# dernasherbrezon/sdr-server

Hardware: AMD Instinct MI355X
Metric: input IQ Msamples/s processed (all clients), 2.016 Msps->48 kHz xlating FIR (higher is better)
Workload: dtype f32; 1 GPU; 1024 clients x 48 kHz off one 2.016 Msps cu8 stream, D=42, 505 taps, 262144-byte blocks (BASELINE configs[3]; N=1: the >=1000-client single-GPU target); clients_total=1024, clients_per_gpu=1024, blocks_per_call=8, mode=optimized, parallelism=single GPU, rccl_ranks=1, feed=xlating_multi (C host)

## Files before the change

sdr-server_amd/csrc/xl_kernels.hip:

```cpp
#include "xl_dev_inline.h"
#include "xl_chain_plan.h"

#include <hip/hip_ext.h>

#include <stdlib.h>

__global__ __launch_bounds__(64) void xl_nco_table_kernel(const XlNcoClient *__restrict__ cl, uint32_t n,
                                                          const float2 *state_in, float2 *state_out,
                                                          float2 *__restrict__ tab, const XlPos pos,
                                                          const uint32_t explicit_K, const uint32_t prio,
                                                          const uint32_t lanes) {
  if (prio == 3) __builtin_amdgcn_s_setprio(3);
  else if (prio == 2) __builtin_amdgcn_s_setprio(2);
  else if (prio == 1) __builtin_amdgcn_s_setprio(1);
  if (threadIdx.x >= lanes) return;
  const uint32_t c = blockIdx.x * lanes + threadIdx.x;
  if (c >= n) return;
  const XlNcoClient k = cl[c];
  const XlBnd bnd = xl_nco_bnd(k, pos, explicit_K);
  asm volatile("" ::: "v255", "a255");
  xl_nco_client_chain<true>(k, bnd, 0u, bnd.K, state_in, state_out, tab);
}

#define XLC_RING 64u
XL_DEV uint32_t xl_lds_off(const void *p) { return (uint32_t)(uintptr_t)(__attribute__((address_space(3))) const char *)p; }
XL_DEV void xl_lds_post(const uint32_t addr, const uint32_t v) { asm volatile("ds_write_b32 %0, %1" ::"v"(addr), "v"(v) : "memory"); }
XL_DEV void xl_lds_post64(const uint32_t addr, const v2f v) { asm volatile("ds_write_b64 %0, %1" ::"v"(addr), "v"(v) : "memory"); }
XL_DEV uint32_t xl_lds_poll(const uint32_t addr) {
  uint32_t v;
  asm volatile("ds_read_b32 %0, %1\n\ts_waitcnt lgkmcnt(0)" : "=v"(v) : "v"(addr) : "memory");
  return v;
}

XL_DEV uint32_t xl_lds_poll3_min(const uint32_t a0, const uint32_t a1, const uint32_t a2) {
  uint32_t v0, v1, v2;
  asm volatile("ds_read_b32 %0, %3\n\tds_read_b32 %1, %4\n\tds_read_b32 %2, %5\n\ts_waitcnt lgkmcnt(0)"
               : "=&v"(v0), "=&v"(v1), "=&v"(v2)
               : "v"(a0), "v"(a1), "v"(a2)
               : "memory");
  v0 = v0 < v1 ? v0 : v1;
  return v0 < v2 ? v0 : v2;
}
XL_DEV uint32_t xl_chain_lim(const uint32_t mn) { return mn >= 0x7FFFFFE0u ? 0xFFFFFFFFu : 2u * mn + XLC_RING; }
XL_DEV uint32_t xl_chain_wait_drained(const uint32_t upto, const uint32_t a0, const uint32_t a1, const uint32_t a2) {
  uint32_t lim = 0u;
  for (uint32_t spin = 0; spin < (1u << 22); ++spin) {
    lim = xl_chain_lim((uint32_t)__builtin_amdgcn_readfirstlane((int)xl_lds_poll3_min(a0, a1, a2)));
    if (upto <= lim) break;
    __builtin_amdgcn_s_sleep(1);
  }
  return lim;
}
XL_DEV uint32_t xl_chain_event(uint32_t ev) {
  const unsigned long long act = __ballot(ev != 0xFFFFFFFFu);
  if (act == 0ull) return 0xFFFFFFFFu;
  const uint32_t first = (uint32_t)__builtin_amdgcn_readlane((int)ev, (int)__ffsll((long long)act) - 1);
  if (__ballot(ev != 0xFFFFFFFFu && ev != first) == 0ull) return first;
#pragma unroll
  for (int sh = 1; sh < 64; sh <<= 1) {
    const uint32_t other = (uint32_t)__shfl_xor((int)ev, sh);
    ev = other < ev ? other : ev;
  }
  return (uint32_t)__builtin_amdgcn_readfirstlane((int)ev);
}

#define XLC_ALIGN ".p2align 6\n\t"
#define XLC_MUL "v_pk_mul_f32 %[t1], %[p], %[inc] op_sel_hi:[1,0]\n\tv_pk_mul_f32 %[t2], %[p], %[inc] op_sel:[0,1] op_sel_hi:[1,1]\n\t"
#define XLC_ADD "v_pk_add_f32 %[p], %[t1], %[t2] op_sel:[0,1] op_sel_hi:[1,0] neg_lo:[0,1]\n\t"
#define XLC_STEP XLC_MUL XLC_ADD
#define XLC_STEP2(I1, I2) XLC_MUL I1 "\n\t" XLC_ADD I2 "\n\t"
#define XLC_STEPS10 XLC_STEP XLC_STEP XLC_STEP XLC_STEP XLC_STEP XLC_STEP XLC_STEP XLC_STEP XLC_STEP XLC_STEP
#define XLC_ANY_LOOP                                                                       \
  "1:\n\t" XLC_MUL "ds_write_b64 %[addr], %[p]\n\t" XLC_ADD                               \
  XLC_STEP2("v_add_u32 %[cnt], 1, %[cnt]", "s_sub_u32 %[todo], %[todo], 1")               \
  XLC_MUL "ds_write_b32 %[paddr], %[cnt]\n\t" XLC_ADD                                     \
  XLC_MUL "v_add_u32 %[off], 0x200, %[off]\n\t" XLC_ADD                                   \
  XLC_MUL "v_and_b32 %[off], 0x7fff, %[off]\n\t" XLC_ADD                                  \
  XLC_STEP2("v_add_u32 %[addr], %[off], %[base]", "s_cmp_lg_u32 %[todo], 0")              \
  XLC_STEPS10 "s_cbranch_scc1 1b\n\t"
#define XLC_B8_LOOP                                                                        \
  "2:\n\t" XLC_E7("0", "512", "1024", "1536", "2048", "2560", "3072")                    \
  XLC_MUL "ds_write_b64 %[addr], %[p] offset:3584\n\t" XLC_ADD                           \
  XLC_STEP2("v_add_u32 %[cnt], 8, %[cnt]", "s_sub_u32 %[todo8], %[todo8], 1")            \
  XLC_MUL "ds_write_b32 %[paddr], %[cnt]\n\t" XLC_ADD                                    \
  XLC_MUL "v_add_u32 %[off], 0x1000, %[off]\n\t" XLC_ADD                                 \
  XLC_MUL "v_and_b32 %[off], 0x7fff, %[off]\n\t" XLC_ADD                                 \
  XLC_STEP2("v_add_u32 %[addr], %[off], %[base]", "s_cmp_lg_u32 %[todo8], 0")            \
  XLC_STEPS10 "s_cbranch_scc1 2b\n\t"
#define XLC_ANY_PART "s_cmp_eq_u32 %[todo], 0\n\ts_cbranch_scc1 3f\n\t" XLC_ANY_LOOP "3:\n\ts_nop 0\n\t"
#define XLC_B8_PART "s_cmp_eq_u32 %[todo8], 0\n\ts_cbranch_scc1 4f\n\t" XLC_B8_LOOP "4:\n\ts_nop 0\n\t"
#define XLC_STEP_LOOP "1:\n\t" XLC_STEP2("s_sub_u32 %[todo], %[todo], 1", "s_cmp_lg_u32 %[todo], 0") "s_cbranch_scc1 1b\n\t"
#define XLC_QENTRY(OFFS) XLC_MUL "ds_write_b64 %[addr], %[p] offset:" OFFS "\n\t" XLC_ADD XLC_STEP XLC_STEP
#define XLC_E(OFFS) XLC_QENTRY(OFFS) XLC_STEP XLC_STEP XLC_STEP XLC_STEPS10
#define XLC_E7(B0, B1, B2, B3, B4, B5, B6) XLC_E(B0) XLC_E(B1) XLC_E(B2) XLC_E(B3) XLC_E(B4) XLC_E(B5) XLC_E(B6)
#define XLC_E8(B0, B1, B2, B3, B4, B5, B6, B7) XLC_E7(B0, B1, B2, B3, B4, B5, B6) XLC_E(B7)
#define XLC_B32_LOOP                                                                                         \
  XLC_E8("0", "512", "1024", "1536", "2048", "2560", "3072", "3584")                                       \
  XLC_E8("4096", "4608", "5120", "5632", "6144", "6656", "7168", "7680")                                   \
  XLC_E8("8192", "8704", "9216", "9728", "10240", "10752", "11264", "11776")                               \
  XLC_E("12288") XLC_E("12800") XLC_E("13312") XLC_E("13824") XLC_E("14336") XLC_E("14848")               \
  XLC_QENTRY("15360")                                                                                      \
  XLC_MUL "ds_read_b32 %[mn], %[an0]\n\t" XLC_ADD                                                           \
  XLC_MUL "ds_read_b32 %[n1], %[an1]\n\t" XLC_ADD                                                           \
  XLC_MUL "ds_read_b32 %[n2], %[an2]\n\t" XLC_ADD XLC_STEPS10                                               \
  XLC_MUL "ds_write_b64 %[addr], %[p] offset:15872\n\t" XLC_ADD                                             \
  XLC_MUL "v_add_u32 %[cnt], 32, %[cnt]\n\t" XLC_ADD "s_sub_u32 %[todo], %[todo], 1\n\t"                    \
  XLC_MUL "ds_write_b32 %[paddr], %[cnt]\n\t" XLC_ADD                                                       \
  XLC_MUL "v_add_u32 %[off], 0x4000, %[off]\n\t" XLC_ADD                                                    \
  XLC_MUL "v_and_b32 %[off], 0x7fff, %[off]\n\t" XLC_ADD                                                    \
  XLC_STEP2("v_add_u32 %[addr], %[off], %[base]", "s_add_u32 %[need], %[need], 16")                         \
  XLC_STEP2("s_waitcnt lgkmcnt(0)", "v_min_u32 %[mn], %[mn], %[n1]")                                        \
  XLC_STEP2("v_min_u32 %[mn], %[mn], %[n2]", "s_nop 0")                                                     \
  XLC_STEP2("v_readfirstlane_b32 %[sm], %[mn]", "s_nop 0")                                                  \
  XLC_STEP2("s_cmp_ge_u32 %[sm], %[need]", "s_cselect_b32 %[st], %[todo], 0")                               \
  XLC_STEP XLC_STEP XLC_STEP XLC_STEP XLC_STEP XLC_STEP
static_assert(XL_PH_STRIDE == 16u && XLC_RING * 64u * 8u == 0x8000u, "the chain wave's asm blocks are written for 16 steps per entry and a 32 KB ring");

__global__ __launch_bounds__(256) void xl_nco_chain_kernel(const XlNcoClient *__restrict__ cl, uint32_t n,
                                                           const float2 *state_in, const XlChainCalls calls,
                                                           XlPos pos, unsigned long long *stats) {
  asm volatile("" ::: "v255", "a255");
  const unsigned long long t_entry = stats ? wall_clock64() : 0ull;
  __shared__ v2f ring[XLC_RING][64];
  __shared__ uint32_t s_emax;
  __shared__ uint32_t s_prod;
  __shared__ uint32_t s_next[3];
  const uint32_t w = __builtin_amdgcn_readfirstlane(threadIdx.x >> 6), lane = threadIdx.x & 63u;
  const uint32_t c = blockIdx.x * 64u + lane;
  const bool have = c < n;
  XlNcoClient k;
  k.incr = make_float2(1.0f, 0.0f);
  k.out_off = 0u, k.slot = 0u, k.D = 1u, k.rem0 = 0u;
  if (have) k = cl[c];
  v2f p = {1.0f, 0.0f};
  if (w == 0 && have) p = (v2f){state_in[k.slot].x, state_in[k.slot].y};
  unsigned long long cyc = 0ull, ticks = 0ull, wfirst = 0ull;
  uint32_t entries = 0u;
  for (uint32_t call = 0; call < calls.n; ++call, pos = xl_grid_next(pos)) {
    float2 *const tab = calls.tab[call];
    float2 *const state_out = calls.state_out[call];
    if (call) __syncthreads();
    XlBnd bnd = xl_nco_bnd(k, pos, 0xFFFFFFFFu);
    if (!have) bnd.K = 0u;
    const uint32_t K = bnd.K, E = (K + XL_PH_STRIDE - 1u) >> XL_PH_SHIFT;
    if (threadIdx.x == 0) {
      s_emax = 0u;
      s_prod = 0u;
      s_next[0] = 0u, s_next[1] = 1u, s_next[2] = 2u;
    }
    __syncthreads();
    if (w == 0 && E > 0u) atomicMax(&s_emax, E);
    __syncthreads();
    const uint32_t Emax = (uint32_t)__builtin_amdgcn_readfirstlane((int)s_emax);
    const uint32_t a_prod = xl_lds_off(&s_prod), a_ring0 = xl_lds_off(&ring[0][0]), a_ring = xl_lds_off(&ring[0][lane]);
    v2f *__restrict__ o = reinterpret_cast<v2f *>(tab) + (k.out_off >> XL_PH_SHIFT);
    if (w == 0) {
      __builtin_amdgcn_s_setprio(3);
      const v2f inc = {k.incr.x, k.incr.y};
      uint32_t nb = xl_bnd_next(bnd, 0u);
      const uint32_t a_n0 = xl_lds_off(&s_next[0]), a_n1 = xl_lds_off(&s_next[1]), a_n2 = xl_lds_off(&s_next[2]);
      const unsigned long long c0 = stats ? clock64() : 0ull, w0 = stats ? wall_clock64() : 0ull;
      unsigned long long t_region = 0ull, t_drain = 0ull, t_b32 = 0ull;
      uint32_t n_drain = 0u, n_b32 = 0u, n_event = 0u, n_runs = 0u;
      uint32_t e = 0;
      uint32_t lim = XLC_RING;
      uint32_t evs = xl_chain_event(0u < K ? (nb < K ? nb : K) : 0xFFFFFFFFu);
      while (e < Emax) {
        uint32_t e_stop = evs == 0u ? 0u : (evs - 1u) >> XL_PH_SHIFT;
        e_stop = e_stop < Emax ? e_stop : Emax;
        if (pos.pad & XL_POS_FMA_STEP) e_stop = e;
        const unsigned long long r0 = stats ? clock64() : 0ull;
        if ((e << XL_PH_SHIFT) < K) {
          const XlChainPlan8 pl = xl_chain_plan8(e, e_stop, XLC_RING, 32u, 8u);
          uint32_t ee = e;
          v2f t1, t2;
#define XLC_COVER_RUN(N1, N8, PARTS)                                                                                         \
  if ((N1) + (N8) != 0u) {                                                                                                   \
    uint32_t todo = (N1), todo8 = (N8);                                                                                      \
    const uint32_t total = todo + 8u * todo8;                                                                                \
    if (ee + total > lim) {                                                                                                  \
      const unsigned long long d0 = stats ? clock64() : 0ull;                                                                \
      lim = xl_chain_wait_drained(ee + total, a_n0, a_n1, a_n2);                                                             \
      if (stats) t_drain += clock64() - d0, ++n_drain;                                                                       \
    }                                                                                                                        \
    uint32_t off = ((ee & (XLC_RING - 1u)) << 9) + lane * (uint32_t)sizeof(v2f);     \
    uint32_t addr = a_ring0 + off, cnt = ee;                                                                                 \
    ee += total;                                                                                                             \
    asm volatile(XLC_ALIGN PARTS                                                                                             \
                 : [p] "+v"(p), [off] "+v"(off), [addr] "+v"(addr), [cnt] "+v"(cnt), [t1] "=&v"(t1), [t2] "=&v"(t2),         \
                   [todo] "+s"(todo), [todo8] "+s"(todo8)                                                                    \
                 : [inc] "v"(inc), [base] "v"(a_ring0), [paddr] "v"(a_prod)                                                  \
                 : "memory", "scc");                                                                                         \
  }
          XLC_COVER_RUN(pl.head1, pl.head8, XLC_ANY_PART XLC_B8_PART);
          for (uint32_t want = pl.blocks; want != 0u;) {
            if (ee + 32u > lim) {
              const unsigned long long d0 = stats ? clock64() : 0ull;
              lim = xl_chain_wait_drained(ee + 32u, a_n0, a_n1, a_n2);
              if (stats) t_drain += clock64() - d0, ++n_drain;
            }
            uint32_t off = ((ee & (XLC_RING - 1u)) << 9) + lane * (uint32_t)sizeof(v2f);
            uint32_t addr = a_ring0 + off, cnt = ee;
            uint32_t left = want, need = (ee >> 1) - 16u, mn, n1, n2, sm, st;
            const unsigned long long b0 = stats ? clock64() : 0ull;
            asm volatile(XLC_ALIGN "1:\n\t" XLC_B32_LOOP "s_cmp_lg_u32 %[st], 0\n\ts_cbranch_scc1 1b\n\t"
                         : [p] "+v"(p), [off] "+v"(off), [addr] "+v"(addr), [cnt] "+v"(cnt), [t1] "=&v"(t1), [t2] "=&v"(t2),
                           [mn] "=&v"(mn), [n1] "=&v"(n1), [n2] "=&v"(n2), [todo] "+s"(left), [need] "+s"(need), [sm] "=&s"(sm),
                           [st] "=&s"(st)
                         : [inc] "v"(inc), [base] "v"(a_ring0), [paddr] "v"(a_prod), [an0] "v"(a_n0), [an1] "v"(a_n1), [an2] "v"(a_n2)
                         : "memory", "scc");
            const uint32_t ran = (want - left) << 5;
            if (stats) t_b32 += clock64() - b0, n_b32 += ran, ++n_runs;
            lim = xl_chain_lim(sm);
            ee += ran;
            want = left;
          }
          XLC_COVER_RUN(pl.tail1, pl.tail8, XLC_B8_PART XLC_ANY_PART);
#undef XLC_COVER_RUN
        }
        if (e_stop > e) e = e_stop;
        if (stats) t_region += clock64() - r0, ++n_event;
        if (e < Emax) {
          if (e + 1u > lim) lim = xl_chain_wait_drained(e + 1u, a_n0, a_n1, a_n2);
          const uint32_t m0 = e << XL_PH_SHIFT;
          if (m0 < K) xl_lds_post64(a_ring + (e & (XLC_RING - 1u)) * 64u * (uint32_t)sizeof(v2f), p);
          xl_lds_post(a_prod, e + 1u);
          uint32_t m = m0;
          if (!(pos.pad & XL_POS_FMA_STEP) && evs - m0 - 1u < XL_PH_STRIDE &&
              __ballot(m0 < K && (nb != evs || m0 + XL_PH_STRIDE > K)) == 0ull && m0 < K) {
            v2f t1, t2;
            uint32_t todo = evs - m0;
            asm volatile(XLC_ALIGN XLC_STEP_LOOP
                         : [p] "+v"(p), [t1] "=&v"(t1), [t2] "=&v"(t2), [todo] "+s"(todo)
                         : [inc] "v"(inc)
                         : "scc");
            p = xl_nco_renorm(p);
            nb = xl_bnd_next(bnd, evs);
            m = evs;
            todo = m0 + XL_PH_STRIDE - evs;
            if (todo != 0u && __ballot(nb <= m0 + XL_PH_STRIDE) == 0ull) {
              asm volatile(XLC_ALIGN XLC_STEP_LOOP
                           : [p] "+v"(p), [t1] "=&v"(t1), [t2] "=&v"(t2), [todo] "+s"(todo)
                           : [inc] "v"(inc)
                           : "scc");
              m = m0 + XL_PH_STRIDE;
            }
          }
          for (; m < m0 + XL_PH_STRIDE && m < K; ++m) {
            p = xl_nco_next_any(p, inc, bnd.flags);
            if (m + 1u == nb) {
              p = xl_nco_renorm(p);
              nb = xl_bnd_next(bnd, m + 1u);
            }
          }
          ++e;
          evs = xl_chain_event((e << XL_PH_SHIFT) < K ? (nb < K ? nb : K) : 0xFFFFFFFFu);
        }
      }
      if (have) state_out[k.slot] = make_float2(p.x, p.y);
      if (stats) {
        cyc += clock64() - c0;
        const unsigned long long w1 = wall_clock64();
        ticks += w1 - w0;
        entries += Emax;
        if (call == 0u) wfirst = w0;
        if (lane == 0u && blockIdx.x < 1024u) {
          stats[8192u + 8u * blockIdx.x + 1u + 2u * call] = w0 - t_entry;
          stats[8192u + 8u * blockIdx.x + 2u + 2u * call] = w1 - t_entry;
        }
        if (lane == 0u && blockIdx.x < 128u) {
          unsigned long long *const sp = stats + 4096u + 32u * blockIdx.x + 8u * call;
          const unsigned long long k0 = clock64(), k1 = clock64(), k2 = clock64(), k3 = clock64(), k4 = clock64();
          (void)k1, (void)k2, (void)k3;
          sp[0] = k0 - c0, sp[1] = t_region, sp[2] = t_drain, sp[3] = t_b32;
          sp[4] = n_drain, sp[5] = n_b32, sp[6] = n_event | ((unsigned long long)n_runs << 32), sp[7] = (k4 - k0) / 4ull;
        }
      }
      continue;
    }
    const uint32_t j = w - 1u;
    const uint32_t a_next = xl_lds_off(&s_next[j]);
    v4f *__restrict__ o4 = reinterpret_cast<v4f *>(o);
    for (uint32_t q = j; 2u * q < Emax; q += 3u) {
      const uint32_t need = 2u * q + 2u < Emax ? 2u * q + 2u : Emax;
      for (uint32_t spin = 0; spin < (1u << 24); ++spin) {
        if (xl_lds_poll(a_prod) >= need) break;
        __builtin_amdgcn_s_sleep(1);
      }
      if (2u * q < E) {
        v2f a, b2 = {0.0f, 0.0f};
        const uint32_t ra = a_ring + ((2u * q) & (XLC_RING - 1u)) * 64u * (uint32_t)sizeof(v2f);
        const uint32_t rb = a_ring + ((2u * q + 1u) & (XLC_RING - 1u)) * 64u * (uint32_t)sizeof(v2f);
        const bool two = 2u * q + 1u < E;
        asm volatile("ds_read_b64 %0, %1" : "=v"(a) : "v"(ra) : "memory");
        if (two) asm volatile("ds_read_b64 %0, %1" : "=v"(b2) : "v"(rb) : "memory");
        asm volatile("s_waitcnt lgkmcnt(0)" ::: "memory");
        if (two) o4[q] = (v4f){a.x, a.y, b2.x, b2.y};
        else o[2u * q] = a;
      }
      xl_lds_post(a_next, q + 3u);
    }
    xl_lds_post(a_next, 0xFFFFFFFFu);
  }
  if (stats) __syncthreads();
  if (stats && threadIdx.x == 0u) {
    if (blockIdx.x < 1024u) {
      stats[8192u + 8u * blockIdx.x] = t_entry;
      stats[8192u + 8u * blockIdx.x + 7u] = wall_clock64() - t_entry;
    }
    stats[4u * blockIdx.x] = cyc;
    stats[4u * blockIdx.x + 1u] = ticks;
    stats[4u * blockIdx.x + 2u] = entries;
    stats[4u * blockIdx.x + 3u] = wfirst;
  }
}

template <int FMT>
XL_DEV void xl_stage_window(const XlFirArgs &a, const uint32_t zero_below, const uint32_t win0, const uint32_t wlen,
                            v2f *__restrict__ win) {
  const uint32_t bd = blockDim.x;
  for (uint32_t j0 = threadIdx.x; j0 < wlen; j0 += 4u * bd) {
    v2f v[4];
    bool ok[4];
#pragma unroll
    for (int u = 0; u < 4; ++u) {
      const uint32_t j = j0 + u * bd;
      const uint32_t s = win0 + j;
      const bool first = s < a.n0;
      ok[u] = j < wlen && s >= zero_below && (first || s - a.n0 < a.n1);
      const void *src = (first || !ok[u]) ? a.in0 : a.in1;
      const uint32_t idx = ok[u] ? (first ? s : s - a.n0) : 0u;
      v[u] = xl_sample(src, FMT, idx);
    }
#pragma unroll
    for (int u = 0; u < 4; ++u) {
      const uint32_t j = j0 + u * bd;
      if (j < wlen) win[j] = ok[u] ? v[u] : (v2f){0.0f, 0.0f};
    }
  }
}

template <int CT, int MODE, bool WIDE>
__global__ __launch_bounds__(64 * XL_NW_MAX) __attribute__((amdgpu_num_sgpr(96))) void xl_fir_kernel(const XlFirArgs a) {
  extern __shared__ __attribute__((aligned(16))) v2f xl_win[];
  const uint32_t OT = a.ota;

  if (blockIdx.x < a.nco_blocks) {
    if (((a.flags >> 4) & 3u) == 3u) __builtin_amdgcn_s_setprio(3);
    else if (((a.flags >> 4) & 3u) == 2u) __builtin_amdgcn_s_setprio(2);
    else if (((a.flags >> 4) & 3u) == 1u) __builtin_amdgcn_s_setprio(1);
    const uint32_t nwave = threadIdx.x >> 6, nlane = threadIdx.x & 63u;
    if (nwave < a.nco_wpw && nlane < XL_NCO_LANES) {
      const unsigned long long t0 = a.trace ? wall_clock64() : 0ull;
      const uint32_t c = (blockIdx.x * a.nco_wpw + nwave) * XL_NCO_LANES + nlane;
      if (c < a.nco_nclients) {
        const XlNcoClient k = a.nco_clients[c];
        const XlBnd bnd = xl_nco_bnd(k, xl_grid_next(a.pos), 0xFFFFFFFFu);
        xl_nco_client_chain<false>(k, bnd, 0u, bnd.K, a.nco_state_in, a.nco_state_out, a.nco_tab);
      }
      if (a.trace && nlane == 0) {
        unsigned long long *tn = a.trace + ((size_t)blockIdx.x * XL_NW_MAX + nwave) * 6;
        tn[0] = t0;
        tn[3] = wall_clock64();
        tn[4] = __builtin_amdgcn_s_getreg((4 << 0) | (0 << 6) | (31 << 11));
        tn[5] = __builtin_amdgcn_s_getreg((20 << 0) | (0 << 6) | (31 << 11));
      }
    }
    return;
  }

  if (!(a.flags & 2u)) __builtin_amdgcn_s_setprio(3);
  const uint32_t b = blockIdx.x - a.nco_blocks;
  const unsigned long long t_entry = a.trace ? wall_clock64() : 0ull;

  const uint32_t roll_blocks = gridDim.x - a.nco_blocks < XL_ROLL_BLOCKS ? gridDim.x - a.nco_blocks : XL_ROLL_BLOCKS;
  if (a.hist_out != nullptr && b < roll_blocks) {
    const uint16_t *__restrict__ h0 = reinterpret_cast<const uint16_t *>(a.in0);
    const uint16_t *__restrict__ h1 = reinterpret_cast<const uint16_t *>(a.in1);
    uint16_t *__restrict__ ho = reinterpret_cast<uint16_t *>(a.hist_out);
    const uint32_t hu = a.hist_units, nu = a.block_units;
    for (uint32_t j = b * blockDim.x + threadIdx.x; j < hu; j += roll_blocks * blockDim.x) {
      const uint32_t sidx = nu + j;
      ho[j] = (sidx < hu) ? h0[sidx] : h1[sidx - hu];
    }
  }
  const uint32_t xcd = b & 7u, idx = b >> 3;
  const uint32_t total = a.ngroups * a.xtiles;
  const uint32_t per = total >> 3, extra = total & 7u;
// ... 131 lines not shown
    if (m < K && lane < OT) {
#pragma unroll
      for (int c = 0; c < CT; ++c) {
        if ((uint32_t)c < ncl) out[t[2 + c] + m] = xl_rotate<MODE>(acc[c].value(), phs[c]);
      }
    }
  }
  if (tr && lane == 0) {
    __builtin_amdgcn_s_waitcnt(0);
    tr[3] = wall_clock64();
  }
}

size_t xl_fir_lds_bytes_ota(uint32_t D, uint32_t Tpad, uint32_t ota) {
  return ((size_t)(ota - 1u) * D + Tpad) * sizeof(v2f);
}

uint32_t xl_fir_pick_ota(uint32_t D, uint32_t Tpad, size_t budget) {
  for (uint32_t ota = 64; ota >= 8; ota >>= 1)
    if (xl_fir_lds_bytes_ota(D, Tpad, ota) <= budget) return ota;
  return 0;
}

template <int CT, int MODE, bool WIDE>
static hipError_t xl_fir_go2(int nw, const XlFirArgs &a, size_t lds, hipStream_t s) {
  static bool attr_done = false;
  if (!attr_done) {
    hipError_t e = hipFuncSetAttribute(reinterpret_cast<const void *>(&xl_fir_kernel<CT, MODE, WIDE>),
                                       hipFuncAttributeMaxDynamicSharedMemorySize, 160 * 1024);
    if (e != hipSuccess) return e;
    attr_done = true;
  }
  const uint32_t nblocks = a.nco_blocks + 8u * ((a.ngroups * a.xtiles + 7u) / 8u);
  if (nblocks == 0) return hipSuccess;
  const size_t need = (size_t)nw * CT * 64u * sizeof(float2);
  if (lds < need) lds = need;
  hipLaunchKernelGGL((xl_fir_kernel<CT, MODE, WIDE>), dim3(nblocks), dim3(64 * nw), lds, s, a);
  return hipGetLastError();
}

template <int CT, int MODE>
static hipError_t xl_fir_go(int nw, const XlFirArgs &a, size_t lds, hipStream_t s) {
  return (a.flags & 1u) ? xl_fir_go2<CT, MODE, true>(nw, a, lds, s) : xl_fir_go2<CT, MODE, false>(nw, a, lds, s);
}

hipError_t xl_launch_fir(int ct, int mode, int nw, const XlFirArgs &a, size_t lds, hipStream_t s) {
  if (lds > 160 * 1024 || nw < 1 || nw > XL_NW_MAX) return hipErrorInvalidValue;
  if (a.ota != 64 && a.ota != 32 && a.ota != 16 && a.ota != 8) return hipErrorInvalidValue;
  switch (ct * 2 + (mode ? 1 : 0)) {
    case 2: return xl_fir_go<1, 0>(nw, a, lds, s);
    case 3: return xl_fir_go<1, 1>(nw, a, lds, s);
    case 4: return xl_fir_go<2, 0>(nw, a, lds, s);
    case 5: return xl_fir_go<2, 1>(nw, a, lds, s);
    case 8: return xl_fir_go<4, 0>(nw, a, lds, s);
    case 9: return xl_fir_go<4, 1>(nw, a, lds, s);
    case 16: return xl_fir_go<8, 0>(nw, a, lds, s);
    case 17: return xl_fir_go<8, 1>(nw, a, lds, s);
    case 18: return xl_fir_go<9, 0>(nw, a, lds, s);
    case 19: return xl_fir_go<9, 1>(nw, a, lds, s);
    case 20: return xl_fir_go<10, 0>(nw, a, lds, s);
    case 21: return xl_fir_go<10, 1>(nw, a, lds, s);
    case 24: return xl_fir_go<12, 0>(nw, a, lds, s);
    case 25: return xl_fir_go<12, 1>(nw, a, lds, s);
    default: return hipErrorInvalidValue;
  }
}

hipError_t xl_launch_nco_table(const XlNcoClient *clients, uint32_t nclients, const float2 *state_in,
                               float2 *state_out, float2 *phtab, XlPos pos, uint32_t explicit_K, uint32_t prio,
                               hipStream_t s) {
  if (nclients == 0) return hipSuccess;
  const uint32_t lanes = XL_NCO_LANES;
  hipLaunchKernelGGL(xl_nco_table_kernel, dim3((nclients + lanes - 1) / lanes), dim3(64), 0, s, clients, nclients,
                     state_in, state_out, phtab, pos, explicit_K, prio, lanes);
  return hipGetLastError();
}

hipError_t xl_launch_nco_chain(const XlNcoClient *clients, uint32_t nclients, const float2 *state_in,
                               const XlChainCalls &calls, XlPos pos, unsigned long long *stats, hipStream_t s,
                               hipEvent_t done) {
  if (calls.n < 1u || calls.n > XL_CHAIN_MAXCALLS) return hipErrorInvalidValue;
  if (nclients == 0) return done ? hipEventRecord(done, s) : hipSuccess;
  if (done)
    hipExtLaunchKernelGGL(xl_nco_chain_kernel, dim3((nclients + 63u) / 64u), dim3(256), 0, s, nullptr, done, 0, clients,
                          nclients, state_in, calls, pos, stats);
  else
    hipLaunchKernelGGL(xl_nco_chain_kernel, dim3((nclients + 63u) / 64u), dim3(256), 0, s, clients, nclients, state_in,
                       calls, pos, stats);
  return hipGetLastError();
}

__global__ void xl_convert_cf32_kernel(const void *__restrict__ raw, int fmt, uint32_t n, v2f *__restrict__ dst) {
  for (uint32_t i = blockIdx.x * blockDim.x + threadIdx.x; i < n; i += gridDim.x * blockDim.x)
    dst[i] = xl_sample(raw, fmt, i);
}

hipError_t xl_launch_convert_cf32(const void *raw, int fmt, uint32_t nsamples, float2 *dst, hipStream_t s) {
  if (nsamples == 0) return hipSuccess;
  const uint32_t blocks = (nsamples + 255) / 256 < 2048 ? (nsamples + 255) / 256 : 2048;
  hipLaunchKernelGGL(xl_convert_cf32_kernel, dim3(blocks), dim3(256), 0, s, raw, fmt, nsamples,
                     reinterpret_cast<v2f *>(dst));
  return hipGetLastError();
}

__global__ void xl_convert_q15_kernel(const void *__restrict__ raw, int fmt, uint32_t n, int16_t *__restrict__ dst) {
  for (uint32_t i = blockIdx.x * blockDim.x + threadIdx.x; i < n; i += gridDim.x * blockDim.x) {
    int32_t v;
    if (fmt == XLF_CU8) {
      v = ((int32_t) reinterpret_cast<const uint8_t *>(raw)[i] - 128) * 256;
    } else if (fmt == XLF_CS8) {
      v = (int32_t) reinterpret_cast<const int8_t *>(raw)[i] * 256;
    } else {
      v = reinterpret_cast<const int16_t *>(raw)[i];
    }
    dst[i] = (int16_t)v;
  }
}

hipError_t xl_launch_convert_q15(const void *raw, int fmt, uint32_t nelems, int16_t *dst, hipStream_t s) {
  if (nelems == 0) return hipSuccess;
  const uint32_t blocks = (nelems + 255) / 256 < 2048 ? (nelems + 255) / 256 : 2048;
  hipLaunchKernelGGL(xl_convert_q15_kernel, dim3(blocks), dim3(256), 0, s, raw, fmt, nelems, dst);
  return hipGetLastError();
}

__global__ __launch_bounds__(1024) void xl_move_down_kernel(uint32_t *buf, uint32_t from_dw, uint32_t count_dw) {
  for (uint32_t base = 0; base < count_dw; base += 1024) {
    const uint32_t i = base + threadIdx.x;
    uint32_t v = 0;
    if (i < count_dw) v = buf[from_dw + i];
    __syncthreads();
    if (i < count_dw) buf[i] = v;
    __syncthreads();
  }
}

hipError_t xl_launch_move_down(void *buf, uint32_t from, uint32_t count, uint32_t elem_bytes, hipStream_t s) {
  if (count == 0 || from == 0) return hipSuccess;
  const uint32_t k = elem_bytes / 4;
  hipLaunchKernelGGL(xl_move_down_kernel, dim3(1), dim3(1024), 0, s, reinterpret_cast<uint32_t *>(buf), from * k,
                     count * k);
  return hipGetLastError();
}

__global__ void xl_update_history_kernel(const uint16_t *__restrict__ hist, const uint16_t *__restrict__ block,
                                         uint32_t h_u, uint32_t n_u, uint16_t *__restrict__ out) {
  for (uint32_t j = blockIdx.x * blockDim.x + threadIdx.x; j < h_u; j += gridDim.x * blockDim.x) {
    const uint32_t s = n_u + j;
    out[j] = (s < h_u) ? hist[s] : block[s - h_u];
  }
}

hipError_t xl_launch_update_history(const void *hist, const void *block, uint32_t h, uint32_t n, uint32_t bps,
                                    void *new_hist, hipStream_t s) {
  if (h == 0) return hipSuccess;
  const uint32_t u = bps / 2;
  const uint32_t hu = h * u, nu = n * u;
  const uint32_t blocks = (hu + 255) / 256 < 256 ? (hu + 255) / 256 : 256;
  hipLaunchKernelGGL(xl_update_history_kernel, dim3(blocks), dim3(256), 0, s, reinterpret_cast<const uint16_t *>(hist),
                     reinterpret_cast<const uint16_t *>(block), hu, nu, reinterpret_cast<uint16_t *>(new_hist));
  return hipGetLastError();
}


XL_DEV uint32_t xl_q15_step(const uint32_t p, const uint32_t a, const uint32_t b) {
  typedef short s2 __attribute__((ext_vector_type(2)));
  const int32_t tr = __builtin_amdgcn_sdot2(__builtin_bit_cast(s2, p), __builtin_bit_cast(s2, a), 0, false);
  const int32_t ti = __builtin_amdgcn_sdot2(__builtin_bit_cast(s2, p), __builtin_bit_cast(s2, b), 0, false);
  return __builtin_bit_cast(uint32_t, __builtin_amdgcn_cvt_pk_i16(tr >> 15, ti >> 15));
}
// ... 197 lines not shown
```

Before: 5.816 million Msamples/s.

## Store NCO chain entries directly to global memory from single-wave blocks

Replaces the 4-wave producer/consumer NCO chain kernel, where one wave generated phasor entries into an LDS ring and three waves drained them to the global table, with a single 64-lane wave per block. That wave issues global_store_dwordx2 directly inside the unrolled rotation asm loops. A large dummy LDS claim keeps occupancy at about one chain wave per CU. This removes LDS ring handshaking, polling, barriers and drain stalls. In exchange, the serial phasor recurrence now waits on global store issue, and coalescing changes because each lane writes its own row.

```diff
diff --git a/sdr-server_amd/csrc/xl_chain_runs.h b/sdr-server_amd/csrc/xl_chain_runs.h
--- /dev/null
+++ b/sdr-server_amd/csrc/xl_chain_runs.h
@@ -0,0 +1,30 @@
+#ifndef XL_CHAIN_RUNS_H_
+#define XL_CHAIN_RUNS_H_
+#include <stdint.h>
+
+#ifndef XL_HD
+#if defined(__HIPCC__) || defined(__CUDACC__)
+#define XL_HD __host__ __device__ static inline
+#else
+#define XL_HD static inline
+#endif
+#endif
+
+typedef struct XlChainRuns {
+  uint32_t runs32;
+  uint32_t runs8;
+  uint32_t singles;
+} XlChainRuns;
+
+XL_HD XlChainRuns xl_chain_runs(uint32_t e, uint32_t e_stop) {
+  XlChainRuns r = {0u, 0u, 0u};
+  uint32_t left;
+  if (e_stop <= e) return r;
+  left = e_stop - e;
+  r.runs32 = left >> 5;
+  r.runs8 = (left & 31u) >> 3;
+  r.singles = left & 7u;
+  return r;
+}
+
+#endif
diff --git a/sdr-server_amd/csrc/xl_kernels.hip b/sdr-server_amd/csrc/xl_kernels.hip
--- a/sdr-server_amd/csrc/xl_kernels.hip
+++ b/sdr-server_amd/csrc/xl_kernels.hip
@@ -1,5 +1,5 @@
 #include "xl_dev_inline.h"
-#include "xl_chain_plan.h"
+#include "xl_chain_runs.h"
 
 #include <hip/hip_ext.h>
 
@@ -22,35 +22,8 @@
   xl_nco_client_chain<true>(k, bnd, 0u, bnd.K, state_in, state_out, tab);
 }
 
-#define XLC_RING 64u
+#define XLC_LDS_CLAIM (96u * 1024u)
 XL_DEV uint32_t xl_lds_off(const void *p) { return (uint32_t)(uintptr_t)(__attribute__((address_space(3))) const char *)p; }
-XL_DEV void xl_lds_post(const uint32_t addr, const uint32_t v) { asm volatile("ds_write_b32 %0, %1" ::"v"(addr), "v"(v) : "memory"); }
-XL_DEV void xl_lds_post64(const uint32_t addr, const v2f v) { asm volatile("ds_write_b64 %0, %1" ::"v"(addr), "v"(v) : "memory"); }
-XL_DEV uint32_t xl_lds_poll(const uint32_t addr) {
-  uint32_t v;
-  asm volatile("ds_read_b32 %0, %1\n\ts_waitcnt lgkmcnt(0)" : "=v"(v) : "v"(addr) : "memory");
-  return v;
-}
-
-XL_DEV uint32_t xl_lds_poll3_min(const uint32_t a0, const uint32_t a1, const uint32_t a2) {
-  uint32_t v0, v1, v2;
-  asm volatile("ds_read_b32 %0, %3\n\tds_read_b32 %1, %4\n\tds_read_b32 %2, %5\n\ts_waitcnt lgkmcnt(0)"
-               : "=&v"(v0), "=&v"(v1), "=&v"(v2)
-               : "v"(a0), "v"(a1), "v"(a2)
-               : "memory");
-  v0 = v0 < v1 ? v0 : v1;
-  return v0 < v2 ? v0 : v2;
-}
-XL_DEV uint32_t xl_chain_lim(const uint32_t mn) { return mn >= 0x7FFFFFE0u ? 0xFFFFFFFFu : 2u * mn + XLC_RING; }
-XL_DEV uint32_t xl_chain_wait_drained(const uint32_t upto, const uint32_t a0, const uint32_t a1, const uint32_t a2) {
-  uint32_t lim = 0u;
-  for (uint32_t spin = 0; spin < (1u << 22); ++spin) {
-    lim = xl_chain_lim((uint32_t)__builtin_amdgcn_readfirstlane((int)xl_lds_poll3_min(a0, a1, a2)));
-    if (upto <= lim) break;
-    __builtin_amdgcn_s_sleep(1);
-  }
-  return lim;
-}
 XL_DEV uint32_t xl_chain_event(uint32_t ev) {
   const unsigned long long act = __ballot(ev != 0xFFFFFFFFu);
   if (act == 0ull) return 0xFFFFFFFFu;
@@ -62,6 +35,16 @@
     ev = other < ev ? other : ev;
   }
   return (uint32_t)__builtin_amdgcn_readfirstlane((int)ev);
+}
+XL_DEV uint32_t xl_chain_emax(uint32_t en) {
+  const uint32_t first = (uint32_t)__builtin_amdgcn_readfirstlane((int)en);
+  if (__ballot(en != first) == 0ull) return first;
+#pragma unroll
+  for (int sh = 1; sh < 64; sh <<= 1) {
+    const uint32_t other = (uint32_t)__shfl_xor((int)en, sh);
+    en = other > en ? other : en;
+  }
+  return (uint32_t)__builtin_amdgcn_readfirstlane((int)en);
 }
 
 #define XLC_ALIGN ".p2align 6\n\t"
@@ -70,62 +53,46 @@
 #define XLC_STEP XLC_MUL XLC_ADD
 #define XLC_STEP2(I1, I2) XLC_MUL I1 "\n\t" XLC_ADD I2 "\n\t"
 #define XLC_STEPS10 XLC_STEP XLC_STEP XLC_STEP XLC_STEP XLC_STEP XLC_STEP XLC_STEP XLC_STEP XLC_STEP XLC_STEP
-#define XLC_ANY_LOOP                                                                       \
-  "1:\n\t" XLC_MUL "ds_write_b64 %[addr], %[p]\n\t" XLC_ADD                               \
-  XLC_STEP2("v_add_u32 %[cnt], 1, %[cnt]", "s_sub_u32 %[todo], %[todo], 1")               \
-  XLC_MUL "ds_write_b32 %[paddr], %[cnt]\n\t" XLC_ADD                                     \
-  XLC_MUL "v_add_u32 %[off], 0x200, %[off]\n\t" XLC_ADD                                   \
-  XLC_MUL "v_and_b32 %[off], 0x7fff, %[off]\n\t" XLC_ADD                                  \
-  XLC_STEP2("v_add_u32 %[addr], %[off], %[base]", "s_cmp_lg_u32 %[todo], 0")              \
-  XLC_STEPS10 "s_cbranch_scc1 1b\n\t"
-#define XLC_B8_LOOP                                                                        \
-  "2:\n\t" XLC_E7("0", "512", "1024", "1536", "2048", "2560", "3072")                    \
-  XLC_MUL "ds_write_b64 %[addr], %[p] offset:3584\n\t" XLC_ADD                           \
-  XLC_STEP2("v_add_u32 %[cnt], 8, %[cnt]", "s_sub_u32 %[todo8], %[todo8], 1")            \
-  XLC_MUL "ds_write_b32 %[paddr], %[cnt]\n\t" XLC_ADD                                    \
-  XLC_MUL "v_add_u32 %[off], 0x1000, %[off]\n\t" XLC_ADD                                 \
-  XLC_MUL "v_and_b32 %[off], 0x7fff, %[off]\n\t" XLC_ADD                                 \
-  XLC_STEP2("v_add_u32 %[addr], %[off], %[base]", "s_cmp_lg_u32 %[todo8], 0")            \
-  XLC_STEPS10 "s_cbranch_scc1 2b\n\t"
-#define XLC_ANY_PART "s_cmp_eq_u32 %[todo], 0\n\ts_cbranch_scc1 3f\n\t" XLC_ANY_LOOP "3:\n\ts_nop 0\n\t"
-#define XLC_B8_PART "s_cmp_eq_u32 %[todo8], 0\n\ts_cbranch_scc1 4f\n\t" XLC_B8_LOOP "4:\n\ts_nop 0\n\t"
+#define XLC_STEPS13 XLC_STEP XLC_STEP XLC_STEP XLC_STEPS10
 #define XLC_STEP_LOOP "1:\n\t" XLC_STEP2("s_sub_u32 %[todo], %[todo], 1", "s_cmp_lg_u32 %[todo], 0") "s_cbranch_scc1 1b\n\t"
-#define XLC_QENTRY(OFFS) XLC_MUL "ds_write_b64 %[addr], %[p] offset:" OFFS "\n\t" XLC_ADD XLC_STEP XLC_STEP
+#define XLC_ST(OFFS) "global_store_dwordx2 %[off], %[p], %[tab] offset:" OFFS "\n\t"
+#define XLC_QENTRY(OFFS) XLC_MUL XLC_ST(OFFS) XLC_ADD XLC_STEP XLC_STEP
 #define XLC_E(OFFS) XLC_QENTRY(OFFS) XLC_STEP XLC_STEP XLC_STEP XLC_STEPS10
 #define XLC_E7(B0, B1, B2, B3, B4, B5, B6) XLC_E(B0) XLC_E(B1) XLC_E(B2) XLC_E(B3) XLC_E(B4) XLC_E(B5) XLC_E(B6)
 #define XLC_E8(B0, B1, B2, B3, B4, B5, B6, B7) XLC_E7(B0, B1, B2, B3, B4, B5, B6) XLC_E(B7)
-#define XLC_B32_LOOP                                                                                         \
-  XLC_E8("0", "512", "1024", "1536", "2048", "2560", "3072", "3584")                                       \
-  XLC_E8("4096", "4608", "5120", "5632", "6144", "6656", "7168", "7680")                                   \
-  XLC_E8("8192", "8704", "9216", "9728", "10240", "10752", "11264", "11776")                               \
-  XLC_E("12288") XLC_E("12800") XLC_E("13312") XLC_E("13824") XLC_E("14336") XLC_E("14848")               \
-  XLC_QENTRY("15360")                                                                                      \
-  XLC_MUL "ds_read_b32 %[mn], %[an0]\n\t" XLC_ADD                                                           \
-  XLC_MUL "ds_read_b32 %[n1], %[an1]\n\t" XLC_ADD                                                           \
-  XLC_MUL "ds_read_b32 %[n2], %[an2]\n\t" XLC_ADD XLC_STEPS10                                               \
-  XLC_MUL "ds_write_b64 %[addr], %[p] offset:15872\n\t" XLC_ADD                                             \
-  XLC_MUL "v_add_u32 %[cnt], 32, %[cnt]\n\t" XLC_ADD "s_sub_u32 %[todo], %[todo], 1\n\t"                    \
-  XLC_MUL "ds_write_b32 %[paddr], %[cnt]\n\t" XLC_ADD                                                       \
-  XLC_MUL "v_add_u32 %[off], 0x4000, %[off]\n\t" XLC_ADD                                                    \
-  XLC_MUL "v_and_b32 %[off], 0x7fff, %[off]\n\t" XLC_ADD                                                    \
-  XLC_STEP2("v_add_u32 %[addr], %[off], %[base]", "s_add_u32 %[need], %[need], 16")                         \
-  XLC_STEP2("s_waitcnt lgkmcnt(0)", "v_min_u32 %[mn], %[mn], %[n1]")                                        \
-  XLC_STEP2("v_min_u32 %[mn], %[mn], %[n2]", "s_nop 0")                                                     \
-  XLC_STEP2("v_readfirstlane_b32 %[sm], %[mn]", "s_nop 0")                                                  \
-  XLC_STEP2("s_cmp_ge_u32 %[sm], %[need]", "s_cselect_b32 %[st], %[todo], 0")                               \
-  XLC_STEP XLC_STEP XLC_STEP XLC_STEP XLC_STEP XLC_STEP
-static_assert(XL_PH_STRIDE == 16u && XLC_RING * 64u * 8u == 0x8000u, "the chain wave's asm blocks are written for 16 steps per entry and a 32 KB ring");
-
-__global__ __launch_bounds__(256) void xl_nco_chain_kernel(const XlNcoClient *__restrict__ cl, uint32_t n,
-                                                           const float2 *state_in, const XlChainCalls calls,
-                                                           XlPos pos, unsigned long long *stats) {
+#define XLC_R32_LOOP                                                                       \
+  "6:\n\t" XLC_E8("0", "8", "16", "24", "32", "40", "48", "56")                          \
+  XLC_E8("64", "72", "80", "88", "96", "104", "112", "120")                              \
+  XLC_E8("128", "136", "144", "152", "160", "168", "176", "184")                         \
+  XLC_E7("192", "200", "208", "216", "224", "232", "240")                                \
+  XLC_MUL XLC_ST("248") XLC_ADD                                                          \
+  XLC_MUL "v_add_u32 %[off], 0x100, %[off]\n\t" XLC_ADD                                  \
+  XLC_STEP2("s_sub_u32 %[n32], %[n32], 1", "s_cmp_lg_u32 %[n32], 0")                     \
+  XLC_STEPS13 "s_cbranch_scc1 6b\n\t"
+#define XLC_R8_LOOP                                                                        \
+  "2:\n\t" XLC_E7("0", "8", "16", "24", "32", "40", "48")                                \
+  XLC_MUL XLC_ST("56") XLC_ADD                                                           \
+  XLC_STEP2("v_add_u32 %[off], 64, %[off]", "s_sub_u32 %[n8], %[n8], 1")                 \
+  XLC_STEP2("s_cmp_lg_u32 %[n8], 0", "s_nop 0")                                          \
+  XLC_STEPS13 "s_cbranch_scc1 2b\n\t"
+#define XLC_R1_LOOP                                                                        \
+  "1:\n\t" XLC_MUL XLC_ST("0") XLC_ADD                                                   \
+  XLC_STEP2("v_add_u32 %[off], 8, %[off]", "s_sub_u32 %[n1], %[n1], 1")                  \
+  XLC_STEP2("s_cmp_lg_u32 %[n1], 0", "s_nop 0")                                          \
+  XLC_STEPS13 "s_cbranch_scc1 1b\n\t"
+#define XLC_R32_PART "s_cmp_eq_u32 %[n32], 0\n\ts_cbranch_scc1 7f\n\t" XLC_R32_LOOP "7:\n\ts_nop 0\n\t"
+#define XLC_R8_PART "s_cmp_eq_u32 %[n8], 0\n\ts_cbranch_scc1 4f\n\t" XLC_R8_LOOP "4:\n\ts_nop 0\n\t"
+#define XLC_R1_PART "s_cmp_eq_u32 %[n1], 0\n\ts_cbranch_scc1 3f\n\t" XLC_R1_LOOP "3:\n\ts_nop 0\n\t"
+static_assert(XL_PH_STRIDE == 16u && sizeof(v2f) == 8u, "the chain wave's asm blocks are written for 16 steps per entry and 8-byte entries");
+
+__global__ __launch_bounds__(64) void xl_nco_chain_kernel(const XlNcoClient *__restrict__ cl, uint32_t n,
+                                                          const float2 *state_in, const XlChainCalls calls,
+                                                          XlPos pos, unsigned long long *stats) {
   asm volatile("" ::: "v255", "a255");
   const unsigned long long t_entry = stats ? wall_clock64() : 0ull;
-  __shared__ v2f ring[XLC_RING][64];
-  __shared__ uint32_t s_emax;
-  __shared__ uint32_t s_prod;
-  __shared__ uint32_t s_next[3];
-  const uint32_t w = __builtin_amdgcn_readfirstlane(threadIdx.x >> 6), lane = threadIdx.x & 63u;
+  __shared__ uint32_t lds_claim[XLC_LDS_CLAIM / sizeof(uint32_t)];
+  asm volatile("" ::"s"(xl_lds_off(lds_claim)));
+  const uint32_t lane = threadIdx.x;
   const uint32_t c = blockIdx.x * 64u + lane;
   const bool have = c < n;
   XlNcoClient k;
@@ -133,177 +100,102 @@
   k.out_off = 0u, k.slot = 0u, k.D = 1u, k.rem0 = 0u;
   if (have) k = cl[c];
   v2f p = {1.0f, 0.0f};
-  if (w == 0 && have) p = (v2f){state_in[k.slot].x, state_in[k.slot].y};
+  if (have) p = (v2f){state_in[k.slot].x, state_in[k.slot].y};
+  const v2f inc = {k.incr.x, k.incr.y};
+  const uint32_t row = (k.out_off >> XL_PH_SHIFT) * (uint32_t)sizeof(v2f);
   unsigned long long cyc = 0ull, ticks = 0ull, wfirst = 0ull;
   uint32_t entries = 0u;
+  __builtin_amdgcn_s_setprio(3);
   for (uint32_t call = 0; call < calls.n; ++call, pos = xl_grid_next(pos)) {
     float2 *const tab = calls.tab[call];
     float2 *const state_out = calls.state_out[call];
-    if (call) __syncthreads();
     XlBnd bnd = xl_nco_bnd(k, pos, 0xFFFFFFFFu);
     if (!have) bnd.K = 0u;
     const uint32_t K = bnd.K, E = (K + XL_PH_STRIDE - 1u) >> XL_PH_SHIFT;
-    if (threadIdx.x == 0) {
-      s_emax = 0u;
-      s_prod = 0u;
-      s_next[0] = 0u, s_next[1] = 1u, s_next[2] = 2u;
-    }
-    __syncthreads();
-    if (w == 0 && E > 0u) atomicMax(&s_emax, E);
-    __syncthreads();
-    const uint32_t Emax = (uint32_t)__builtin_amdgcn_readfirstlane((int)s_emax);
-    const uint32_t a_prod = xl_lds_off(&s_prod), a_ring0 = xl_lds_off(&ring[0][0]), a_ring = xl_lds_off(&ring[0][lane]);
+    const uint32_t Emax = xl_chain_emax(E);
     v2f *__restrict__ o = reinterpret_cast<v2f *>(tab) + (k.out_off >> XL_PH_SHIFT);
-    if (w == 0) {
-      __builtin_amdgcn_s_setprio(3);
-      const v2f inc = {k.incr.x, k.incr.y};
-      uint32_t nb = xl_bnd_next(bnd, 0u);
-      const uint32_t a_n0 = xl_lds_off(&s_next[0]), a_n1 = xl_lds_off(&s_next[1]), a_n2 = xl_lds_off(&s_next[2]);
-      const unsigned long long c0 = stats ? clock64() : 0ull, w0 = stats ? wall_clock64() : 0ull;
-      unsigned long long t_region = 0ull, t_drain = 0ull, t_b32 = 0ull;
-      uint32_t n_drain = 0u, n_b32 = 0u, n_event = 0u, n_runs = 0u;
-      uint32_t e = 0;
-      uint32_t lim = XLC_RING;
-      uint32_t evs = xl_chain_event(0u < K ? (nb < K ? nb : K) : 0xFFFFFFFFu);
-      while (e < Emax) {
-        uint32_t e_stop = evs == 0u ? 0u : (evs - 1u) >> XL_PH_SHIFT;
-        e_stop = e_stop < Emax ? e_stop : Emax;
-        if (pos.pad & XL_POS_FMA_STEP) e_stop = e;
-        const unsigned long long r0 = stats ? clock64() : 0ull;
-        if ((e << XL_PH_SHIFT) < K) {
-          const XlChainPlan8 pl = xl_chain_plan8(e, e_stop, XLC_RING, 32u, 8u);
-          uint32_t ee = e;
+    const unsigned long long tab_base = (unsigned long long)(uintptr_t)tab;
+    uint32_t nb = xl_bnd_next(bnd, 0u);
+    const unsigned long long c0 = stats ? clock64() : 0ull, w0 = stats ? wall_clock64() : 0ull;
+    unsigned long long t_region = 0ull, t_runs = 0ull;
+    uint32_t n_ents = 0u, n_event = 0u, n_runs = 0u;
+    uint32_t e = 0;
+    uint32_t evs = xl_chain_event(0u < K ? (nb < K ? nb : K) : 0xFFFFFFFFu);
+    while (e < Emax) {
+      uint32_t e_stop = evs == 0u ? 0u : (evs - 1u) >> XL_PH_SHIFT;
+      e_stop = e_stop < Emax ? e_stop : Emax;
+      if (pos.pad & XL_POS_FMA_STEP) e_stop = e;
+      const unsigned long long r0 = stats ? clock64() : 0ull;
+      if (e_stop > e && (e << XL_PH_SHIFT) < K) {
+        const XlChainRuns rn = xl_chain_runs(e, e_stop);
+        uint32_t n32 = rn.runs32, n8 = rn.runs8, n1 = rn.singles;
+        uint32_t off = row + e * (uint32_t)sizeof(v2f);
+        v2f t1, t2;
+        const unsigned long long b0 = stats ? clock64() : 0ull;
+        asm volatile(XLC_ALIGN XLC_R32_PART XLC_R8_PART XLC_R1_PART
+                     : [p] "+v"(p), [off] "+v"(off), [t1] "=&v"(t1), [t2] "=&v"(t2), [n32] "+s"(n32), [n8] "+s"(n8), [n1] "+s"(n1)
+                     : [inc] "v"(inc), [tab] "s"(tab_base)
+                     : "memory", "scc");
+        if (stats) t_runs += clock64() - b0, n_ents += e_stop - e, ++n_runs;
+      }
+      if (e_stop > e) e = e_stop;
+      if (stats) t_region += clock64() - r0, ++n_event;
+      if (e < Emax) {
+        const uint32_t m0 = e << XL_PH_SHIFT;
+        if (m0 < K) o[e] = p;
+        uint32_t m = m0;
+        if (!(pos.pad & XL_POS_FMA_STEP) && evs - m0 - 1u < XL_PH_STRIDE &&
+            __ballot(m0 < K && (nb != evs || m0 + XL_PH_STRIDE > K)) == 0ull && m0 < K) {
           v2f t1, t2;
-#define XLC_COVER_RUN(N1, N8, PARTS)                                                                                         \
-  if ((N1) + (N8) != 0u) {                                                                                                   \
-    uint32_t todo = (N1), todo8 = (N8);                                                                                      \
-    const uint32_t total = todo + 8u * todo8;                                                                                \
-    if (ee + total > lim) {                                                                                                  \
-      const unsigned long long d0 = stats ? clock64() : 0ull;                                                                \
-      lim = xl_chain_wait_drained(ee + total, a_n0, a_n1, a_n2);                                                             \
-      if (stats) t_drain += clock64() - d0, ++n_drain;                                                                       \
-    }                                                                                                                        \
-    uint32_t off = ((ee & (XLC_RING - 1u)) << 9) + lane * (uint32_t)sizeof(v2f);     \
-    uint32_t addr = a_ring0 + off, cnt = ee;                                                                                 \
-    ee += total;                                                                                                             \
-    asm volatile(XLC_ALIGN PARTS                                                                                             \
-                 : [p] "+v"(p), [off] "+v"(off), [addr] "+v"(addr), [cnt] "+v"(cnt), [t1] "=&v"(t1), [t2] "=&v"(t2),         \
-                   [todo] "+s"(todo), [todo8] "+s"(todo8)                                                                    \
-                 : [inc] "v"(inc), [base] "v"(a_ring0), [paddr] "v"(a_prod)                                                  \
-                 : "memory", "scc");                                                                                         \
-  }
-          XLC_COVER_RUN(pl.head1, pl.head8, XLC_ANY_PART XLC_B8_PART);
-          for (uint32_t want = pl.blocks; want != 0u;) {
-            if (ee + 32u > lim) {
-              const unsigned long long d0 = stats ? clock64() : 0ull;
-              lim = xl_chain_wait_drained(ee + 32u, a_n0, a_n1, a_n2);
-              if (stats) t_drain += clock64() - d0, ++n_drain;
-            }
-            uint32_t off = ((ee & (XLC_RING - 1u)) << 9) + lane * (uint32_t)sizeof(v2f);
-            uint32_t addr = a_ring0 + off, cnt = ee;
-            uint32_t left = want, need = (ee >> 1) - 16u, mn, n1, n2, sm, st;
-            const unsigned long long b0 = stats ? clock64() : 0ull;
-            asm volatile(XLC_ALIGN "1:\n\t" XLC_B32_LOOP "s_cmp_lg_u32 %[st], 0\n\ts_cbranch_scc1 1b\n\t"
-                         : [p] "+v"(p), [off] "+v"(off), [addr] "+v"(addr), [cnt] "+v"(cnt), [t1] "=&v"(t1), [t2] "=&v"(t2),
-                           [mn] "=&v"(mn), [n1] "=&v"(n1), [n2] "=&v"(n2), [todo] "+s"(left), [need] "+s"(need), [sm] "=&s"(sm),
-                           [st] "=&s"(st)
-                         : [inc] "v"(inc), [base] "v"(a_ring0), [paddr] "v"(a_prod), [an0] "v"(a_n0), [an1] "v"(a_n1), [an2] "v"(a_n2)
-                         : "memory", "scc");
-            const uint32_t ran = (want - left) << 5;
-            if (stats) t_b32 += clock64() - b0, n_b32 += ran, ++n_runs;
-            lim = xl_chain_lim(sm);
-            ee += ran;
-            want = left;
-          }
-          XLC_COVER_RUN(pl.tail1, pl.tail8, XLC_B8_PART XLC_ANY_PART);
-#undef XLC_COVER_RUN
-        }
-        if (e_stop > e) e = e_stop;
-        if (stats) t_region += clock64() - r0, ++n_event;
-        if (e < Emax) {
-          if (e + 1u > lim) lim = xl_chain_wait_drained(e + 1u, a_n0, a_n1, a_n2);
-          const uint32_t m0 = e << XL_PH_SHIFT;
-          if (m0 < K) xl_lds_post64(a_ring + (e & (XLC_RING - 1u)) * 64u * (uint32_t)sizeof(v2f), p);
-          xl_lds_post(a_prod, e + 1u);
-          uint32_t m = m0;
-          if (!(pos.pad & XL_POS_FMA_STEP) && evs - m0 - 1u < XL_PH_STRIDE &&
-              __ballot(m0 < K && (nb != evs || m0 + XL_PH_STRIDE > K)) == 0ull && m0 < K) {
-            v2f t1, t2;
-            uint32_t todo = evs - m0;
+          uint32_t todo = evs - m0;
+          asm volatile(XLC_ALIGN XLC_STEP_LOOP
+                       : [p] "+v"(p), [t1] "=&v"(t1), [t2] "=&v"(t2), [todo] "+s"(todo)
+                       : [inc] "v"(inc)
+                       : "scc");
+          p = xl_nco_renorm(p);
+          nb = xl_bnd_next(bnd, evs);
+          m = evs;
+          todo = m0 + XL_PH_STRIDE - evs;
+          if (todo != 0u && __ballot(nb <= m0 + XL_PH_STRIDE) == 0ull) {
             asm volatile(XLC_ALIGN XLC_STEP_LOOP
                          : [p] "+v"(p), [t1] "=&v"(t1), [t2] "=&v"(t2), [todo] "+s"(todo)
                          : [inc] "v"(inc)
                          : "scc");
+            m = m0 + XL_PH_STRIDE;
+          }
+        }
+        for (; m < m0 + XL_PH_STRIDE && m < K; ++m) {
+          p = xl_nco_next_any(p, inc, bnd.flags);
+          if (m + 1u == nb) {
             p = xl_nco_renorm(p);
-            nb = xl_bnd_next(bnd, evs);
-            m = evs;
-            todo = m0 + XL_PH_STRIDE - evs;
-            if (todo != 0u && __ballot(nb <= m0 + XL_PH_STRIDE) == 0ull) {
-              asm volatile(XLC_ALIGN XLC_STEP_LOOP
-                           : [p] "+v"(p), [t1] "=&v"(t1), [t2] "=&v"(t2), [todo] "+s"(todo)
-                           : [inc] "v"(inc)
-                           : "scc");
-              m = m0 + XL_PH_STRIDE;
-            }
+            nb = xl_bnd_next(bnd, m + 1u);
           }
-          for (; m < m0 + XL_PH_STRIDE && m < K; ++m) {
-            p = xl_nco_next_any(p, inc, bnd.flags);
-            if (m + 1u == nb) {
-              p = xl_nco_renorm(p);
-              nb = xl_bnd_next(bnd, m + 1u);
-            }
-          }
-          ++e;
-          evs = xl_chain_event((e << XL_PH_SHIFT) < K ? (nb < K ? nb : K) : 0xFFFFFFFFu);
         }
-      }
-      if (have) state_out[k.slot] = make_float2(p.x, p.y);
-      if (stats) {
-        cyc += clock64() - c0;
-        const unsigned long long w1 = wall_clock64();
-        ticks += w1 - w0;
-        entries += Emax;
-        if (call == 0u) wfirst = w0;
-        if (lane == 0u && blockIdx.x < 1024u) {
-          stats[8192u + 8u * blockIdx.x + 1u + 2u * call] = w0 - t_entry;
-          stats[8192u + 8u * blockIdx.x + 2u + 2u * call] = w1 - t_entry;
-        }
-        if (lane == 0u && blockIdx.x < 128u) {
-          unsigned long long *const sp = stats + 4096u + 32u * blockIdx.x + 8u * call;
-          const unsigned long long k0 = clock64(), k1 = clock64(), k2 = clock64(), k3 = clock64(), k4 = clock64();
-          (void)k1, (void)k2, (void)k3;
-          sp[0] = k0 - c0, sp[1] = t_region, sp[2] = t_drain, sp[3] = t_b32;
-          sp[4] = n_drain, sp[5] = n_b32, sp[6] = n_event | ((unsigned long long)n_runs << 32), sp[7] = (k4 - k0) / 4ull;
-        }
-      }
-      continue;
-    }
-    const uint32_t j = w - 1u;
-    const uint32_t a_next = xl_lds_off(&s_next[j]);
-    v4f *__restrict__ o4 = reinterpret_cast<v4f *>(o);
-    for (uint32_t q = j; 2u * q < Emax; q += 3u) {
-      const uint32_t need = 2u * q + 2u < Emax ? 2u * q + 2u : Emax;
-      for (uint32_t spin = 0; spin < (1u << 24); ++spin) {
-        if (xl_lds_poll(a_prod) >= need) break;
-        __builtin_amdgcn_s_sleep(1);
-      }
-      if (2u * q < E) {
-        v2f a, b2 = {0.0f, 0.0f};
-        const uint32_t ra = a_ring + ((2u * q) & (XLC_RING - 1u)) * 64u * (uint32_t)sizeof(v2f);
-        const uint32_t rb = a_ring + ((2u * q + 1u) & (XLC_RING - 1u)) * 64u * (uint32_t)sizeof(v2f);
-        const bool two = 2u * q + 1u < E;
-        asm volatile("ds_read_b64 %0, %1" : "=v"(a) : "v"(ra) : "memory");
-        if (two) asm volatile("ds_read_b64 %0, %1" : "=v"(b2) : "v"(rb) : "memory");
-        asm volatile("s_waitcnt lgkmcnt(0)" ::: "memory");
-        if (two) o4[q] = (v4f){a.x, a.y, b2.x, b2.y};
-        else o[2u * q] = a;
-      }
-      xl_lds_post(a_next, q + 3u);
-    }
-    xl_lds_post(a_next, 0xFFFFFFFFu);
-  }
-  if (stats) __syncthreads();
-  if (stats && threadIdx.x == 0u) {
+        ++e;
+        evs = xl_chain_event((e << XL_PH_SHIFT) < K ? (nb < K ? nb : K) : 0xFFFFFFFFu);
+      }
+    }
+    if (have) state_out[k.slot] = make_float2(p.x, p.y);
+    if (stats) {
+      cyc += clock64() - c0;
+      const unsigned long long w1 = wall_clock64();
+      ticks += w1 - w0;
+      entries += Emax;
+      if (call == 0u) wfirst = w0;
+      if (lane == 0u && blockIdx.x < 1024u) {
+        stats[8192u + 8u * blockIdx.x + 1u + 2u * call] = w0 - t_entry;
+        stats[8192u + 8u * blockIdx.x + 2u + 2u * call] = w1 - t_entry;
+      }
+      if (lane == 0u && blockIdx.x < 128u) {
+        unsigned long long *const sp = stats + 4096u + 32u * blockIdx.x + 8u * call;
+        const unsigned long long k0 = clock64(), k1 = clock64(), k2 = clock64(), k3 = clock64(), k4 = clock64();
+        (void)k1, (void)k2, (void)k3;
+        sp[0] = k0 - c0, sp[1] = t_region, sp[2] = 0ull, sp[3] = t_runs;
+        sp[4] = 0ull, sp[5] = n_ents, sp[6] = n_event | ((unsigned long long)n_runs << 32), sp[7] = (k4 - k0) / 4ull;
+      }
+    }
+  }
+  if (stats && lane == 0u) {
     if (blockIdx.x < 1024u) {
       stats[8192u + 8u * blockIdx.x] = t_entry;
       stats[8192u + 8u * blockIdx.x + 7u] = wall_clock64() - t_entry;
@@ -601,10 +493,10 @@
   if (calls.n < 1u || calls.n > XL_CHAIN_MAXCALLS) return hipErrorInvalidValue;
   if (nclients == 0) return done ? hipEventRecord(done, s) : hipSuccess;
   if (done)
-    hipExtLaunchKernelGGL(xl_nco_chain_kernel, dim3((nclients + 63u) / 64u), dim3(256), 0, s, nullptr, done, 0, clients,
+    hipExtLaunchKernelGGL(xl_nco_chain_kernel, dim3((nclients + 63u) / 64u), dim3(64), 0, s, nullptr, done, 0, clients,
                           nclients, state_in, calls, pos, stats);
   else
-    hipLaunchKernelGGL(xl_nco_chain_kernel, dim3((nclients + 63u) / 64u), dim3(256), 0, s, clients, nclients, state_in,
+    hipLaunchKernelGGL(xl_nco_chain_kernel, dim3((nclients + 63u) / 64u), dim3(64), 0, s, clients, nclients, state_in,
                        calls, pos, stats);
   return hipGetLastError();
 }
```

New measurement: 5.865 million Msamples/s, median of 6. No clear change (+0.8%).
